# ArtoriasAbyssslayer/HashModNFFBanks-IDR

Hardware: AMD Instinct MI355X
Metric: rays/sec fwd+bwd (hash+SDF MLP) (higher is better)
Workload: dtype f32; 1 GPU; DTU-shaped synthetic uniform-sphere rays, MultiResHash L=16 T=2^19 F=2 (BASELINE.json configs[1]), full IDR training step (forward + IDRLoss + backward + clip + Adam), weights held at the geometric initialisation (lr = 0): the SURVEY.md 8(d) workload; grid_config=C2, rays_per_gpu=2048, global_rays=2048, parallelism=single GPU, world=1, ranks_seen=1, step=HIP-graph captured static-shape step

## Files before the change

### hashmodnffbanks_idr_amd/csrc/hm_trace.hip

```cpp
#include "hm_common.h"
#include "hm_trace_host.h"

#include <stdlib.h>
#include <string.h>

namespace {

constexpr int kTB = 256;

#include "hm_trace_dev.h"

__global__ __launch_bounds__(kTB) void trace_init_kernel(TraceArgs a) {
    const int64_t i = (int64_t)blockIdx.x * kTB + threadIdx.x;
    if (i >= a.n) return;
    trace_init_ray(a, i, a.w.cnt + C_ROUND0, 0);
}

__global__ __launch_bounds__(kTB) void trace_advance_kernel(TraceArgs a, int round) {
    const int64_t i = (int64_t)blockIdx.x * kTB + threadIdx.x;
    if (i >= a.n) return;
    trace_advance_ray(a, i, a.w.cnt + C_ROUND0 + round, 0);
}

__global__ __launch_bounds__(kTB) void trace_finalize_kernel(TraceArgs a) {
    const int64_t i = (int64_t)blockIdx.x * kTB + threadIdx.x;
    if (i >= a.n) return;
    const TraceWs &w = a.w;
    if (w.stage[i] != ST_DONE) atomicAdd(w.cnt + C_UNFINISHED, 1);
    const float t_s = w.t_s[i], t_e = w.t_e[i];
    a.out_mask[i] = t_s < t_e;
    a.out_t[i] = t_s;
    float px = 0.0f, py = 0.0f, pz = 0.0f;
    if (a.hit[i] || w.cnt[C_ANY_LIVE]) along(a, i, t_s, px, py, pz);
    a.out_pts[i * 3] = px; a.out_pts[i * 3 + 1] = py; a.out_pts[i * 3 + 2] = pz;
    const bool samp = w.live_s[i] != 0;
    w.is_samp[i] = samp;
    if (samp) w.list_samp[atomicAdd(w.cnt + C_NSAMP, 1)] = (int32_t)i;
}

__global__ __launch_bounds__(kTB) void ray_samples_kernel(TraceArgs a, const int32_t *list, int c_n, int c_npts,
                                                          const float *lo_arr, const float *hi_arr,
                                                          const float *fr, int c_base, int per_ray) {
    const int64_t gid = (int64_t)blockIdx.x * kTB + threadIdx.x;
    const TraceWs &w = a.w;
    const int32_t n_list = w.cnt[c_n];
    const int64_t base = c_base == -2 ? a.sel_off : (c_base >= 0 ? w.cnt[c_base] : 0);
    if (gid == 0) {
        w.cnt[c_npts] = n_list * per_ray;
        if (c_base != -2) w.cnt[C_BIG_PTS] = (int32_t)base + n_list * per_ray;
    }
    const int64_t m = gid / per_ray;
    if (m >= n_list) return;
    int s = (int)(gid - m * per_ray);
    if (per_ray < a.n_steps && s == per_ray - 1) s = a.n_steps - 1;
    const int64_t i = list[m];
    const float lo = lo_arr[i], hi = hi_arr[i];
    const float t = __fadd_rn(lo, __fmul_rn(fr[s], __fsub_rn(hi, lo)));
    float px, py, pz;
    along(a, i, t, px, py, pz);
    const int64_t o = base + gid;
    w.pts[o * 3] = px; w.pts[o * 3 + 1] = py; w.pts[o * 3 + 2] = pz;
}

__global__ __launch_bounds__(kTB) void sampler_head_kernel(TraceArgs a) {
    const int64_t m = (int64_t)blockIdx.x * kTB + threadIdx.x;
    const TraceWs &w = a.w;
    if (m >= w.cnt[C_NSAMP]) return;
    const int64_t i = w.list_samp[m];
    const float *v = w.vals + m * (a.head + 1);
    bool neg = false;
    for (int s = 0; s < a.head; ++s) neg = neg || (v[s] < 0.0f);
    const bool resolved = neg && a.obj[i] != 0;
    w.tail_slot[m] = resolved ? -1 : atomicAdd(w.cnt + C_NSAMP2, 1);
}

__global__ __launch_bounds__(kTB) void sampler_tail_points_kernel(TraceArgs a) {
    const int64_t gid = (int64_t)blockIdx.x * kTB + threadIdx.x;
    const TraceWs &w = a.w;
    const int per = a.n_steps - a.head - 1;
    if (gid == 0) {
        w.cnt[C_TAIL_PTS] = w.cnt[C_NSAMP2] * per;
        w.cnt[C_NSAMP_PTS] = w.cnt[C_HEAD_PTS] + w.cnt[C_NSAMP2] * per;
    }
    const int64_t m = gid / per;
    if (m >= w.cnt[C_NSAMP]) return;
    const int32_t q = w.tail_slot[m];
    if (q < 0) return;
    const int j = (int)(gid - m * per);
    const int64_t i = w.list_samp[m];
    const float lo = w.t_s[i], hi = w.t_e[i];
    const float t = __fadd_rn(lo, __fmul_rn(a.fracs[a.head + j], __fsub_rn(hi, lo)));
    float px, py, pz;
    along(a, i, t, px, py, pz);
    const int64_t o = a.tail_off + (int64_t)q * per + j;
    w.pts[o * 3] = px; w.pts[o * 3 + 1] = py; w.pts[o * 3 + 2] = pz;
}

__global__ __launch_bounds__(kTB) void sampler_reduce_kernel(TraceArgs a) {
    const int64_t m = (int64_t)blockIdx.x * kTB + threadIdx.x;
    const TraceWs &w = a.w;
    if (m >= w.cnt[C_NSAMP]) return;
    const int64_t i = w.list_samp[m];
    const int n = a.n_steps;
    const bool lazy = a.head > 0;
    const int32_t tq = lazy ? w.tail_slot[m] : 0;
    const float *v_head = lazy ? w.vals + m * (a.head + 1) : w.vals + m * n;
    const float *v_tail = lazy ? w.vals + a.tail_off + (int64_t)(tq < 0 ? 0 : tq) * (n - a.head - 1) - a.head : v_head;
    const int head = a.head;
    auto v = [&](int s) -> float {
        if (!lazy) return v_head[s];
        if (s < head) return v_head[s];
        return s == n - 1 ? v_head[head] : v_tail[s];
    };
    const int n_scan = (lazy && tq < 0) ? head : n;
    int first = 0, amin = 0, bad = 0;
    float best_tmp = 0.0f, best_v = 0.0f;
    auto visit = [&](int s, float x) {
        bad += !isfinite(x);
        const float sg = (x > 0.0f) ? 1.0f : ((x < 0.0f) ? -1.0f : 0.0f);
        const float tmp = sg * (float)(n - s);
        if (s == 0 || tmp < best_tmp) { best_tmp = tmp; first = s; }
        if (s == 0 || x < best_v) { best_v = x; amin = s; }
    };
    if (!lazy && (n & 3) == 0 && (reinterpret_cast<uintptr_t>(v_head) & 15u) == 0) {
        const float4 *row = reinterpret_cast<const float4 *>(v_head);
#pragma unroll 5
        for (int g4 = 0; g4 < n / 4; ++g4) {
            const float4 x4 = row[g4];
            visit(4 * g4, x4.x); visit(4 * g4 + 1, x4.y); visit(4 * g4 + 2, x4.z); visit(4 * g4 + 3, x4.w);
        }
    } else {
        for (int s = 0; s < n_scan; ++s) visit(s, v(s));
    }
    const float lo = w.t_s[i], hi = w.t_e[i];
    auto t_at = [&](int s) { return __fadd_rn(lo, __fmul_rn(a.fracs[s], __fsub_rn(hi, lo))); };
    const float v_first = v(first);
    const bool net_hit = v_first < 0.0f;
    const bool true_obj = a.obj[i] != 0;
    const int pick = (true_obj && net_hit) ? first : amin;
    float t_out = t_at(pick);
    float px, py, pz;
    along(a, i, t_out, px, py, pz);
    a.out_mask[i] = net_hit;
    const bool sec = a.training ? (net_hit && true_obj) : net_hit;
    if (sec) {
        const int lo_idx = first > 0 ? first - 1 : n - 1;
        const float z_hi = t_at(first), v_hi = v_first, z_lo = t_at(lo_idx), v_lo = v(lo_idx);
        if (lazy && tq < 0 && lo_idx == n - 1 && !isfinite(v_lo)) ++bad;
        const float z = secant_z(v_lo, v_hi, z_lo, z_hi);
        const int32_t q = atomicAdd(w.cnt + C_NSEC, 1);
        w.list_sec[q] = (int32_t)i;
        w.z_lo[q] = z_lo; w.z_hi[q] = z_hi; w.v_lo[q] = v_lo; w.v_hi[q] = v_hi; w.z[q] = z;
        if (a.n_secant == 0) {
            t_out = z;
            along(a, i, z, px, py, pz);
        }
    }
    if (bad) atomicAdd(w.cnt + C_NONFINITE, bad);
    a.out_t[i] = t_out;
    w.t_s[i] = t_out;
    a.out_pts[i * 3] = px; a.out_pts[i * 3 + 1] = py; a.out_pts[i * 3 + 2] = pz;
}

__global__ __launch_bounds__(kTB) void secant_points_kernel(TraceArgs a) {
    const int64_t q = (int64_t)blockIdx.x * kTB + threadIdx.x;
    const TraceWs &w = a.w;
    if (q >= w.cnt[C_NSEC]) return;
    float px, py, pz;
    along(a, w.list_sec[q], w.z[q], px, py, pz);
    w.pts[q * 3] = px; w.pts[q * 3 + 1] = py; w.pts[q * 3 + 2] = pz;
}

__global__ __launch_bounds__(kTB) void secant_advance_kernel(TraceArgs a, int last) {
    const int64_t q = (int64_t)blockIdx.x * kTB + threadIdx.x;
    if (q >= a.w.cnt[C_NSEC]) return;
    secant_advance_ray(a, q, last);
}

__global__ __launch_bounds__(kTB) void tail_prepare_kernel(TraceArgs a) {
    const int64_t i = (int64_t)blockIdx.x * kTB + threadIdx.x;
    if (i >= a.n) return;
    const TraceWs &w = a.w;
    const bool net = a.out_mask[i] != 0, obj = a.obj[i] != 0, samp = w.is_samp[i] != 0, hit = a.hit[i] != 0;
    const bool in_mask = !net && obj && !samp;
    const bool out_mask = !obj && !samp;
    if (!(in_mask || out_mask)) return;
    if (!hit) {
        const float *c = a.cam + (i / a.rays_per_image) * 3;
        const float *d = a.dirs + i * 3;
        const float dot = __fmaf_rn(d[2], c[2], __fmaf_rn(d[1], c[1], __fmul_rn(d[0], c[0])));
        const float t = -dot;
        float px, py, pz;
        along(a, i, t, px, py, pz);
        a.out_t[i] = t;
        w.t_s[i] = t;
        a.out_pts[i * 3] = px; a.out_pts[i * 3 + 1] = py; a.out_pts[i * 3 + 2] = pz;
        return;
    }
    if (net && out_mask) w.t_min[i] = w.t_s[i];
    w.list_sel[atomicAdd(w.cnt + C_NSEL, 1)] = (int32_t)i;
}

__global__ __launch_bounds__(kTB) void closest_reduce_kernel(TraceArgs a) {
    const int64_t m = (int64_t)blockIdx.x * kTB + threadIdx.x;
    const TraceWs &w = a.w;
    if (m >= w.cnt[C_NSEL]) return;
    const int64_t i = w.list_sel[m];
    const int n = a.n_steps;
    const float *v = w.vals + (a.sel_off >= 0 ? a.sel_off : (int64_t)w.cnt[a.head > 0 ? C_HEAD_PTS : C_NSAMP_PTS]) +
                     m * n;
    int amin = 0, bad = !isfinite(v[0]);
    float best = v[0];
    if ((n & 3) == 0 && (reinterpret_cast<uintptr_t>(v) & 15u) == 0) {
        const float4 *row = reinterpret_cast<const float4 *>(v);
        auto visit = [&](int s, float x) {
            if (s == 0) return;
            bad += !isfinite(x);
            if (x < best) { best = x; amin = s; }
        };
#pragma unroll 5
        for (int g4 = 0; g4 < n / 4; ++g4) {
            const float4 x4 = row[g4];
            visit(4 * g4, x4.x); visit(4 * g4 + 1, x4.y); visit(4 * g4 + 2, x4.z); visit(4 * g4 + 3, x4.w);
        }
    } else {
        for (int s = 1; s < n; ++s) {
            bad += !isfinite(v[s]);
            if (v[s] < best) { best = v[s]; amin = s; }
        }
    }
    if (bad) atomicAdd(w.cnt + C_NONFINITE, bad);
    const float lo = w.t_min[i], hi = w.t_max[i];
    const float t = __fadd_rn(__fmul_rn(a.steps_u[amin], __fsub_rn(hi, lo)), lo);
    float px, py, pz;
    along(a, i, t, px, py, pz);
    a.out_t[i] = t;
    a.out_pts[i * 3] = px; a.out_pts[i * 3 + 1] = py; a.out_pts[i * 3 + 2] = pz;
}

constexpr int kGuardRows = kTB / 64;
template <class V, class S, class O>
__device__ __forceinline__ void guard_mark_row(const TraceArgs &a, int lane, int n, bool signs, bool min_rule,
                                               bool true_obj, bool all, bool own_approx, bool other_approx, int c_ref,
                                               V val, S slot, O own) {
    const float tau = kGuardTau;
    const int kNone = 1 << 30;
    auto unc = [&](float x) { return !isfinite(x) || fabsf(x) <= tau; };
    int c = kNone;
    float m = INFINITY;
    for (int s = lane; s < n; s += 64) {
        const float x = val(s);
        if (signs && c == kNone && x < -tau) c = s;
        if (isfinite(x) && x < m) m = x;
    }
    for (int d = 32; d > 0; d >>= 1) {
        c = min(c, __shfl_xor(c, d));
        m = fminf(m, __shfl_xor(m, d));
    }
    const bool use_min = min_rule && (!signs || !true_obj || c == kNone);
    const float lim = m + 2.0f * tau;
    auto marked = [&](int s, float x, float xn) -> bool {
        if (!(own(s) ? own_approx : other_approx)) return false;
        if (all && own(s)) return true;
        if (!isfinite(x)) return true;
        if (use_min && x <= lim) return true;
        if (!signs) return false;
        if (fabsf(x) <= tau || s == c) return true;
        const int nx = s + 1 == n ? 0 : s + 1;
        return nx <= c && (nx == c || unc(xn));
    };
    auto mark_of = [&](int s) -> bool { return s < n && marked(s, val(s), val(s + 1 == n ? 0 : s + 1)); };
    int n_mark = 0;
    for (int s0 = 0; s0 < n; s0 += 64) n_mark += __popcll(__ballot(mark_of(s0 + lane)));
    if (n_mark == 0) return;
    int k0 = 0;
    if (lane == 0) k0 = atomicAdd(a.w.cnt + c_ref, n_mark);
    int64_t k = __shfl(k0, 0);
    for (int s0 = 0; s0 < n; s0 += 64) {
        const int s = s0 + lane;
        const bool mk = mark_of(s);
        const unsigned long long b = __ballot(mk);
        if (mk) {
            const int64_t kk = k + __popcll(b & ((1ull << lane) - 1ull));
            const int64_t o = slot(s);
            a.w.ref_slot[kk] = (int32_t)o;
            a.w.ref_pts[kk * 3] = a.w.pts[o * 3]; a.w.ref_pts[kk * 3 + 1] = a.w.pts[o * 3 + 1];
            a.w.ref_pts[kk * 3 + 2] = a.w.pts[o * 3 + 2];
        }
        k += __popcll(b);
    }
}

__global__ __launch_bounds__(kTB) void guard_select_sampler_kernel(TraceArgs a, int pass, int c_live, int c_live2,
                                                                   int64_t min_live, int c_ref) {
    const int64_t m = (int64_t)blockIdx.x * kGuardRows + (threadIdx.x >> 6);
    const int lane = threadIdx.x & 63;
    const TraceWs &w = a.w;
    if (m >= w.cnt[C_NSAMP]) return;
    const bool approx = w.cnt[c_live] >= min_live, approx2 = c_live2 >= 0 && w.cnt[c_live2] >= min_live;
    if (!approx && !approx2) return;
    const bool all = *w.guard == kGuardTripped;
    const bool true_obj = a.obj[w.list_samp[m]] != 0;
    const int n = a.n_steps, head = a.head;
    if (pass == 1) {
        const int row = head > 0 ? head + 1 : n;
        const int64_t base = m * row;
        guard_mark_row(a, lane, row, true, head == 0, true_obj, all, true, false, c_ref,
                       [&](int s) { return w.vals[base + s]; }, [&](int s) { return base + s; }, [](int) { return true; });
        return;
    }
    const int32_t tq = w.tail_slot[m];
    if (tq < 0) return;
    const int64_t b_head = m * (head + 1), b_tail = a.tail_off + (int64_t)tq * (n - head - 1) - head;
    auto slot = [&](int s) -> int64_t { return s < head ? b_head + s : (s == n - 1 ? b_head + head : b_tail + s); };
    guard_mark_row(a, lane, n, true, true, true_obj, all, approx, approx2, c_ref, [&](int s) { return w.vals[slot(s)]; },
                   slot, [&](int s) { return s >= head && s != n - 1; });
}

__global__ __launch_bounds__(kTB) void guard_select_closest_kernel(TraceArgs a, int c_live, int64_t min_live, int c_ref) {
    const int64_t m = (int64_t)blockIdx.x * kGuardRows + (threadIdx.x >> 6);
    const int lane = threadIdx.x & 63;
    const TraceWs &w = a.w;
    if (m >= w.cnt[C_NSEL] || w.cnt[c_live] < min_live) return;
    const int n = a.n_steps;
    const int64_t base = (a.sel_off >= 0 ? a.sel_off : (int64_t)w.cnt[a.head > 0 ? C_HEAD_PTS : C_NSAMP_PTS]) + m * n;
    guard_mark_row(a, lane, n, false, true, false, *w.guard == kGuardTripped, true, false, c_ref,
                   [&](int s) { return w.vals[base + s]; },
                   [&](int s) { return base + s; }, [](int) { return true; });
}

__global__ __launch_bounds__(kTB) void guard_patch_kernel(TraceArgs a, int c_ref) {
    const int64_t k = (int64_t)blockIdx.x * kTB + threadIdx.x;
    const TraceWs &w = a.w;
    const int32_t n_ref = w.cnt[c_ref];
    if (k == 0 && n_ref > 0) atomicAdd(w.cnt + C_GUARD_REFINED, n_ref);
    if (k >= n_ref) return;
    const int64_t o = w.ref_slot[k];
    const float e = w.ref_vals[k], ap = w.vals[o];
    if (isfinite(e) && isfinite(ap)) {
        const float d = fabsf(ap - e);
        if (d > 0.0f) atomicMax(w.cnt + C_GUARD_MAXDEV, __float_as_int(d));
        if (d > kGuardTrip) *w.guard = kGuardTripped;
    }
    w.vals[o] = e;
}

__global__ __launch_bounds__(kTB) void guard_noise_kernel(float *vals, int64_t off, const int32_t *n_live, int64_t min_live,
                                                          float amp, int nan_k) {
    const int64_t g = (int64_t)blockIdx.x * kTB + threadIdx.x;
    const int64_t n = *n_live;
    if (n < min_live || g >= n) return;
    const int64_t o = off + g;
    if (nan_k > 0) {
        if (o % nan_k == 0) vals[o] = ((o / nan_k) & 1) ? INFINITY : NAN;
        return;
    }
    uint32_t h = (uint32_t)o * 2654435761u;
    h ^= h >> 15; h *= 2246822519u; h ^= h >> 13;
    const float u = (float)(h >> 8) * (2.0f / 16777216.0f) - 1.0f;
    vals[o] = __fadd_rn(vals[o], __fmul_rn(amp, u));
}

__global__ void count_evals_kernel(int32_t *cnt, int rounds, int n_secant) {
    if (threadIdx.x != 0 || blockIdx.x != 0) return;
    int64_t tot = 0;
    for (int r = 0; r < rounds && r < 64; ++r) tot += cnt[C_ROUND0 + r];
    tot += cnt[C_NSAMP_PTS] + (int64_t)cnt[C_NSEC] * n_secant + cnt[C_NSEL_PTS];
    cnt[C_EVALS] = (int32_t)tot;
}

constexpr float *TraceWs::*kRayFloats[] = {&TraceWs::t_s,   &TraceWs::t_e,   &TraceWs::t_min, &TraceWs::t_max, &TraceWs::cur_s,
                                           &TraceWs::cur_e, &TraceWs::nxt_s, &TraceWs::nxt_e, &TraceWs::z_lo,  &TraceWs::z_hi,
                                           &TraceWs::v_lo,  &TraceWs::v_hi,  &TraceWs::z};
constexpr int32_t *TraceWs::*kRayInts[] = {&TraceWs::slot_s,   &TraceWs::slot_e,   &TraceWs::list_samp,
                                           &TraceWs::list_sec, &TraceWs::list_sel, &TraceWs::tail_slot};
constexpr uint8_t *TraceWs::*kRayBytes[] = {&TraceWs::live_s, &TraceWs::live_e, &TraceWs::stage,
                                            &TraceWs::it,     &TraceWs::k,      &TraceWs::is_samp};
template <class T, size_t K>
void carve_rays(HmCarve &c, TraceWs &w, T *TraceWs::*const (&members)[K], int64_t n) {
    T *p = c.take<T>((int64_t)K * n);
    for (size_t k = 0; k < K; ++k) w.*members[k] = p + (p ? (int64_t)k * n : 0);
}

constexpr int64_t kWsHeader = 256;
constexpr int kWsRegions = 3;

struct TraceLayout { TraceWs w; float *emb_ws; int64_t bytes; };
TraceLayout trace_layout(void *ws, int64_t n, int n_steps, int emb_width, bool guard) {
    TraceLayout L;
    TraceWs &w = L.w;
    HmCarve c(ws);
    w.cap = n * (n_steps > 2 ? n_steps : 2);
    w.guard = c.take<int32_t>(kWsHeader / (int64_t)sizeof(int32_t));
    carve_rays(c, w, kRayFloats, n);
    carve_rays(c, w, kRayInts, n);
    carve_rays(c, w, kRayBytes, n);
    w.pts = c.take<float>(kWsRegions * 3 * w.cap);
    w.vals = c.take<float>(kWsRegions * w.cap);
    w.cnt = c.take<int32_t>(C_COUNT);
    L.emb_ws = c.take<float>((int64_t)emb_width * w.cap);
    w.ref_pts = c.take<float>(guard ? 5 * w.cap : 0);
    w.ref_vals = w.ref_pts + (ws ? 3 * w.cap : 0);
    w.ref_slot = reinterpret_cast<int32_t *>(w.ref_vals + (ws ? w.cap : 0));
    L.bytes = c.bytes;
    return L;
}
int nffb_emb_width(int n_levels) { return 3 + 8 + 8 * n_levels; }

struct TraceSwitches {
    int overlap, chain_tiles, chain_tail;
    int tail_first;
    float noise_amp; int noise_nan;
};
TraceSwitches trace_switches() {
    const auto num = [](const char *name, int unset) {
        const char *e = getenv(name);
        return e ? atoi(e) : unset;
    };
    TraceSwitches s = {num("HM_TRACE_OVERLAP", -1), num("HM_TRACE_POOL_CHAIN_TILES", -1), num("HM_TRACE_CHAIN_TAIL", -1),
                       num("HM_TRACE_TAIL_FIRST", 0), 0.0f, 0};
    const char *e = getenv("HM_TRACE_GUARD_NOISE");
    if (e && strncmp(e, "nan:", 4) == 0) s.noise_nan = atoi(e + 4) > 0 ? atoi(e + 4) : 0;
    else if (e) { const double f_ = atof(e); if (f_ > 0.0 && f_ < 1.0) s.noise_amp = (float)(f_ * kGuardTau); }
    return s;
}

using TracePlan = hm_trace_plan_info;

TracePlan trace_plan(const hm_trace_cfg &cfg, int64_t n_rays, int tile_points, bool has_nffb, const TraceSwitches &sw) {
    TracePlan P = {};
    const bool guard = cfg.coarse_bf16 == 3;
    const int n_sec = cfg.n_secant_steps;
    const bool overlap_shape = sw.overlap != 0 && cfg.training && !has_nffb && tile_points == 0 && n_sec > 0 && n_rays <= kSdfSmall;
    const bool fill = overlap_shape && cfg.coarse_bf16 == 0;
    const bool cosched = guard && overlap_shape && sw.overlap != 1;
    const bool pooled = cosched && sw.overlap != 2;
    P.sequence = fill ? HM_TRACE_SEQ_FILL : pooled ? HM_TRACE_SEQ_GUARD_POOLED : cosched ? HM_TRACE_SEQ_GUARD_COSCHED
                 : guard ? HM_TRACE_SEQ_GUARD_SERIAL : HM_TRACE_SEQ_JOINT;
    P.sel_own = fill || (guard && overlap_shape);
    P.head = (cfg.sampler_head >= 1 && cfg.sampler_head + 1 < cfg.n_steps) ? cfg.sampler_head : 0;
    P.per_ray = P.head > 0 ? P.head + 1 : cfg.n_steps;
    P.c_first = P.head > 0 ? (int)C_HEAD_PTS : (int)C_NSAMP_PTS;
    const int tail_want = sw.chain_tail >= 0 ? sw.chain_tail : kTraceChainTail;
    P.k_tail = (pooled && tail_want > 0 && n_sec > tail_want) ? tail_want : 0;
    P.chain_tiles = pooled ? trace_chain_tiles(n_sec, sw.chain_tiles >= 0 ? sw.chain_tiles : -1) : 0;
    P.c_ref2 = (pooled && P.head > 0) ? (int)C_GUARD_N2 : -1;
    P.guard_min = tile_points == 0 ? kSdfSmall + 1 : 1;
    if (guard) { P.noise_amp = sw.noise_amp; P.noise_nan = sw.noise_nan; }
    const int64_t cap = n_rays * (cfg.n_steps > 2 ? cfg.n_steps : 2);
    P.march_rounds = 1 + cfg.sphere_tracing_iters * (1 + cfg.line_step_iters);
    P.march_tail = !has_nffb && (tile_points == 0 || tile_points == 16) && cap >= ((n_rays + 7) / 8) * 16 &&
                   cfg.line_step_iters > 0;
    P.march_launched = P.march_tail ? 1 + cfg.sphere_tracing_iters : P.march_rounds;
    if (P.march_tail && sw.tail_first >= 1 && sw.tail_first < P.march_launched) P.march_launched = sw.tail_first;
    if (n_sec == 0) P.secant = HM_TRACE_SECANT_NONE;
    else if (fill || cosched) P.secant = HM_TRACE_SECANT_IN_SEQUENCE;
    else if (!has_nffb && (tile_points == 0 || tile_points == 4 || tile_points == 8 || tile_points == 16) &&
             (tile_points != 0 || n_rays <= kSdfSmall))
        P.secant = HM_TRACE_SECANT_PERSISTENT;
    else P.secant = HM_TRACE_SECANT_PER_ITERATION;
    P.scan_rule = P.secant == HM_TRACE_SECANT_PERSISTENT && P.sel_own;
    return P;
}

struct TraceRun {
    HmTraceCtx cx; const hm_trace_cfg *cfg;
    TracePlan P; TraceArgs a;
    float *emb_ws;
    int emb_width;

    int c_samp() const { return P.sel_own ? P.c_first : (int)C_BIG_PTS; }
    int c_sel() const { return P.sel_own ? (int)C_NSEL_PTS : (int)C_BIG_PTS; }
    int64_t n_scan() const { return a.n * a.n_steps; }
    int64_t n_tail() const { return a.n * (a.n_steps - a.head - 1); }

    template <class K, class... A>
    void launch(K kernel, int64_t threads, A... args) {
        hipLaunchKernelGGL(kernel, dim3((unsigned)((threads + kTB - 1) / kTB)), dim3(kTB), 0, as_stream(cx.stream), args...);
    }
    template <class K, class... A> void per_ray(K kernel, A... args) { launch(kernel, a.n, a, args...); }
    template <class K, class... A> void per_row(K kernel, A... args) { launch(kernel, a.n * (kTB / kGuardRows), a, args...); }

    int eval(int64_t off, int64_t capacity, const int32_t *n_dev, int mode = 0) {
        const float *p = a.w.pts + off * 3;
        float *v = a.w.vals + off;
        const int64_t run_min = kSdfSmall + 1;
        const int tile = mode ? -1 : cx.tile_points;
        if (cx.nffb) {
            HM_TRY(hm_nffb_fwd(cx.desc, cx.nffb, p, capacity, cx.table, cx.B_fourier, emb_ws, emb_width, cx.frac_mode, n_dev,
                               cx.stream));
            HM_TRY(hm_sdf_fwd_emb(cx.mlp, emb_ws, emb_width, emb_width, capacity, v, 1, 1, tile, n_dev, 0, cx.stream));
            if (!mode) return HM_OK;
            return mode == 2 ? hm_sdf_fwd_emb_split(cx.mlp, emb_ws, emb_width, emb_width, capacity, v, 1, n_dev, run_min, cx.stream)
                             : hm_sdf_fwd_emb_bf16(cx.mlp, emb_ws, emb_width, emb_width, capacity, v, 1, n_dev, run_min, cx.stream);
        }
        if (mode == 3 && cx.tile_points != 0)
            return hm_sdf_fwd_split(cx.desc, cx.mlp, p, capacity, cx.table, cx.B_fourier, v, 1, cx.frac_mode, n_dev, 1, cx.stream);
        HM_TRY(hm_sdf_fwd(cx.desc, cx.mlp, p, capacity, cx.table, cx.B_fourier, v, 1, 1, cx.frac_mode, tile, n_dev, 0, cx.stream));
        if (!mode) return HM_OK;
        return mode >= 2 ? hm_sdf_fwd_split(cx.desc, cx.mlp, p, capacity, cx.table, cx.B_fourier, v, 1, cx.frac_mode, n_dev, run_min,
                                            cx.stream)
                         : hm_sdf_fwd_bf16(cx.desc, cx.mlp, p, capacity, cx.table, cx.B_fourier, v, 1, cx.frac_mode, n_dev, run_min,
                                           cx.stream);
    }
    int coarse(int64_t off, int64_t capacity, int c_live) { return eval(off, capacity, a.w.cnt + c_live, cfg->coarse_bf16); }

    void first_pass_points() {
        if (cfg->training) per_ray(tail_prepare_kernel);
        launch(ray_samples_kernel, a.n * P.per_ray, a, a.w.list_samp, (int)C_NSAMP, P.c_first, a.w.t_s, a.w.t_e, a.fracs, -1,
               P.per_ray);
        if (cfg->training)
            launch(ray_samples_kernel, n_scan(), a, a.w.list_sel, (int)C_NSEL, (int)C_NSEL_PTS, a.w.t_min, a.w.t_max, a.steps_u,
                   P.sel_own ? -2 : P.c_first, a.n_steps);
    }
    void second_pass_points() {
        per_ray(sampler_head_kernel);
        launch(sampler_tail_points_kernel, n_scan(), a);
    }

    void noise(int64_t off, int64_t capacity, int c_live) {
        if (P.noise_amp > 0.0f || P.noise_nan > 0)
            launch(guard_noise_kernel, capacity, a.w.vals, off, a.w.cnt + c_live, P.guard_min, P.noise_amp, P.noise_nan);
    }
    void select_sampler(int pass, int c_live, int c_live2, int c_ref) {
        per_row(guard_select_sampler_kernel, pass, c_live, c_live2, P.guard_min, c_ref);
    }
    void select_closest(int c_live, int c_ref) { per_row(guard_select_closest_kernel, c_live, P.guard_min, c_ref); }
    int refine(int c_ref, bool quarter = false) {
        return hm_sdf_fwd(cx.desc, cx.mlp, a.w.ref_pts, a.w.cap, cx.table, cx.B_fourier, a.w.ref_vals, 1, 1, cx.frac_mode,
                          cx.tile_points == 0 ? (quarter ? HM_SDF_TILE64_QUARTER : 64) : cx.tile_points, a.w.cnt + c_ref, 0,
                          cx.stream);
    }
    int refine_beside_scan(int which) {
        return hm_trace_refine_scan(&cx, &a, C_GUARD_N1, P.c_ref2, which, a.sel_off, n_scan(), P.chain_tiles);
    }
    void patch(int c_ref) { launch(guard_patch_kernel, a.w.cap, a, c_ref); }
    int second_pass() {
        if (a.head == 0) return HM_OK;
        second_pass_points();
        HM_TRY(coarse(a.tail_off, n_tail(), C_TAIL_PTS));
        if (cfg->coarse_bf16 != 3) return HM_OK;
        noise(a.tail_off, n_tail(), C_TAIL_PTS);
        select_sampler(2, C_TAIL_PTS, c_samp(), C_GUARD_N2);
        HM_TRY(P.c_ref2 >= 0 ? refine_beside_scan(1) : refine(C_GUARD_N2));
        patch(C_GUARD_N2);
        return HM_OK;
    }
    int sampler_beside_scan() {
        HM_TRY(coarse(0, n_scan(), c_samp()));
        noise(0, n_scan(), c_samp());
        select_sampler(1, c_samp(), -1, C_GUARD_N1);
        HM_TRY(refine_beside_scan(0));
        patch(C_GUARD_N1);
        HM_TRY(second_pass());
        per_ray(sampler_reduce_kernel);
        per_ray(secant_points_kernel);
        return HM_OK;
    }
    template <class F>
    int closest_rows_own_list(F refine_launch) {
        noise(a.sel_off, n_scan(), C_NSEL_PTS);
        select_closest(C_NSEL_PTS, C_GUARD_NC);
        HM_TRY(refine_launch());
        patch(C_GUARD_NC);
        per_ray(closest_reduce_kernel);
        return HM_OK;
    }
    int secant_beside_list(int it_first, int n_iters, int quarter) {
        return hm_trace_scan_secant(&cx, &a, it_first, n_iters, a.n_secant, quarter, a.w.ref_pts, a.w.ref_vals, a.w.cap,
                                    C_GUARD_NC, 0, -1, 0, -1, 0);
    }
    int reduce_and_secant() {
        per_ray(sampler_reduce_kernel);
        if (P.secant == HM_TRACE_SECANT_NONE) return HM_OK;
        per_ray(secant_points_kernel);
        if (P.secant == HM_TRACE_SECANT_PERSISTENT) return hm_trace_secant_persistent(&cx, &a, a.n_secant, P.scan_rule);
        for (int s = 0; s < a.n_secant; ++s) {
            HM_TRY(eval(0, a.n, a.w.cnt + C_NSEC));
            per_ray(secant_advance_kernel, s == a.n_secant - 1 ? 1 : 0);
        }
        return HM_OK;
    }

    int march() {
        per_ray(trace_init_kernel);
        for (int r = 0; r < P.march_launched; ++r) {
            HM_TRY(eval(0, 2 * a.n, a.w.cnt + C_ROUND0 + r));
            per_ray(trace_advance_kernel, r + 1 < 64 ? r + 1 : 63);
        }
        if (P.march_tail) HM_TRY(hm_trace_march_tail(&cx, &a, P.march_launched, P.march_rounds));
        per_ray(trace_finalize_kernel);
        return HM_OK;
    }

    int seq_joint() {
        HM_TRY(coarse(0, n_scan(), C_BIG_PTS));
        if (cfg->training) per_ray(closest_reduce_kernel);
        HM_TRY(second_pass());
        return reduce_and_secant();
    }
    int seq_fill() {
        int grid_p1 = 0, grid_p2 = 0;
        const float *x_fill = a.w.pts + a.sel_off * 3;
        float *out_fill = a.w.vals + a.sel_off;
        HM_TRY(hm_sdf_fwd_fill(&cx, a.w.pts, n_scan(), a.w.vals, a.w.cnt + P.c_first, x_fill, out_fill, a.w.cnt + C_NSEL_PTS,
                               nullptr, 0, &grid_p1));
        if (a.head > 0) {
            second_pass_points();
            HM_TRY(hm_sdf_fwd_fill(&cx, a.w.pts + a.tail_off * 3, n_tail(), a.w.vals + a.tail_off, a.w.cnt + C_TAIL_PTS, x_fill,
                                   out_fill, a.w.cnt + C_NSEL_PTS, a.w.cnt + P.c_first, grid_p1, &grid_p2));
        }
        per_ray(sampler_reduce_kernel);
        per_ray(secant_points_kernel);
        HM_TRY(hm_trace_scan_secant(&cx, &a, 0, a.n_secant, a.n_secant, 0, x_fill, out_fill, n_scan(), C_NSEL_PTS, 1, P.c_first,
                                    grid_p1, C_TAIL_PTS, grid_p2));
        per_ray(closest_reduce_kernel);
        return HM_OK;
    }
    int seq_guard_serial() {
        HM_TRY(coarse(0, n_scan(), c_samp()));
        if (P.sel_own) HM_TRY(coarse(a.sel_off, n_scan(), c_sel()));
        noise(0, n_scan(), c_samp());
        if (P.sel_own) noise(a.sel_off, n_scan(), c_sel());
        select_sampler(1, c_samp(), -1, C_GUARD_N1);
        if (cfg->training) select_closest(c_sel(), C_GUARD_N1);
        HM_TRY(refine(C_GUARD_N1));
        patch(C_GUARD_N1);
        if (cfg->training) per_ray(closest_reduce_kernel);
        HM_TRY(second_pass());
        return reduce_and_secant();
    }
    int seq_guard_cosched() {
        HM_TRY(sampler_beside_scan());
        return closest_rows_own_list([&] { return secant_beside_list(0, a.n_secant, 0); });
    }
    int seq_guard_pooled() {
        const int n_front = a.n_secant - P.k_tail;
        HM_TRY(sampler_beside_scan());
        HM_TRY(hm_trace_split_scan_secant(&cx, &a, 0, n_front, a.n_secant, C_GUARD_N1, P.c_ref2, a.sel_off, n_scan(),
                                          P.chain_tiles));
        return closest_rows_own_list(
            [&] { return P.k_tail > 0 ? secant_beside_list(n_front, P.k_tail, 1) : refine(C_GUARD_NC, true); });
    }

    int run(int32_t *stats_out) {
        hm_zero_u32_async(a.w.cnt, C_COUNT, as_stream(cx.stream));
        HM_TRY(march());
        first_pass_points();
        switch (P.sequence) {
        case HM_TRACE_SEQ_FILL: HM_TRY(seq_fill()); break;
        case HM_TRACE_SEQ_GUARD_SERIAL: HM_TRY(seq_guard_serial()); break;
        case HM_TRACE_SEQ_GUARD_COSCHED: HM_TRY(seq_guard_cosched()); break;
        case HM_TRACE_SEQ_GUARD_POOLED: HM_TRY(seq_guard_pooled()); break;
        default: HM_TRY(seq_joint()); break;
        }
        hipLaunchKernelGGL(count_evals_kernel, dim3(1), dim3(64), 0, as_stream(cx.stream), a.w.cnt, P.march_rounds + 1, a.n_secant);
        if (stats_out)
            hipLaunchKernelGGL(hm_copy_u32_kernel, dim3(1), dim3(64), 0, as_stream(cx.stream), reinterpret_cast<uint32_t *>(stats_out),
                               reinterpret_cast<const uint32_t *>(a.w.cnt + C_NSAMP), 16);
        HM_CHECK_LAUNCH("hm_trace_forward");
        return HM_OK;
    }
};

}

extern "C" {

int64_t hm_trace_workspace_bytes(int64_t n_rays, const hm_trace_cfg *cfg) {
    if (n_rays < 0 || !cfg || cfg->n_steps < 1) return hm_fail(HM_ERR_INVALID, "hm_trace_workspace_bytes: bad argument");
    return trace_layout(nullptr, n_rays, cfg->n_steps, 0, cfg->coarse_bf16 == 3).bytes;
}

int hm_trace_guard_clear(void *workspace, int64_t workspace_bytes, void *stream) {
    HM_CHECK_ARG(workspace && workspace_bytes >= kWsHeader, "hm_trace_guard_clear: no workspace");
    hm_zero_u32_async(reinterpret_cast<int32_t *>(workspace), kWsHeader / sizeof(int32_t), as_stream(stream));
    HM_CHECK_LAUNCH("hm_trace_guard_clear");
    return HM_OK;
}

int hm_trace_guard_tolerances(float *tau, float *tau_trip) {
    HM_CHECK_ARG(tau && tau_trip, "hm_trace_guard_tolerances: NULL pointer");
    *tau = kGuardTau;
    *tau_trip = kGuardTrip;
    return HM_OK;
}

int64_t hm_trace_workspace_bytes_nffb(int64_t n_rays, const hm_trace_cfg *cfg, int n_levels) {
    if (n_rays < 0 || !cfg || cfg->n_steps < 1 || n_levels < 1 || n_levels > HM_MAX_LEVELS)
        return hm_fail(HM_ERR_INVALID, "hm_trace_workspace_bytes_nffb: bad argument");
    return trace_layout(nullptr, n_rays, cfg->n_steps, nffb_emb_width(n_levels), false).bytes;
}

int hm_diag_trace_plan(int64_t n_rays, const hm_trace_cfg *cfg, int tile_points, int has_nffb, hm_trace_plan_info *info) {
    HM_CHECK_ARG(n_rays >= 0 && cfg && info && cfg->n_steps >= 2, "hm_diag_trace_plan: bad argument");
    *info = trace_plan(*cfg, n_rays, tile_points, has_nffb != 0, trace_switches());
    return HM_OK;
}

static int trace_forward_impl(const HmTraceCtx &cx, const hm_trace_cfg *cfg, const float *cam_loc, const float *ray_dirs,
                              const uint8_t *object_mask, const float *t_sphere, const uint8_t *hit_mask, int64_t n_rays,
                              int64_t rays_per_image, const float *sampler_fracs, const float *steps_u, float *out_points,
                              uint8_t *out_net_mask, float *out_dists, void *workspace, int64_t workspace_bytes,
                              int32_t *stats_out) {
    HM_CHECK_ARG(cx.desc && cx.mlp && cfg, "hm_trace_forward: NULL descriptor");
    HM_CHECK_ARG(n_rays >= 0 && rays_per_image >= 1, "hm_trace_forward: bad ray counts");
    HM_CHECK_ARG(cfg->n_steps >= 2 && cfg->n_steps <= 4096, "hm_trace_forward: n_steps out of range");
    HM_CHECK_ARG(cfg->sphere_tracing_iters >= 0 && cfg->sphere_tracing_iters <= 15 && cfg->line_step_iters >= 0 &&
                     cfg->line_step_iters <= 3 &&
                     1 + cfg->sphere_tracing_iters * (1 + cfg->line_step_iters) <= 64,
                 "hm_trace_forward: too many march rounds (sphere_tracing_iters <= 15, line_step_iters <= 3)");
    HM_CHECK_ARG(cfg->n_secant_steps >= 0 && cfg->n_secant_steps <= 64, "hm_trace_forward: n_secant_steps out of range");
    if (n_rays == 0) return HM_OK;
    HM_CHECK_ARG(n_rays * (int64_t)cfg->n_steps < (1ll << 31), "hm_trace_forward: too many rays for one call");
    HM_CHECK_ARG(cx.table && cx.B_fourier && cam_loc && ray_dirs && object_mask && t_sphere && hit_mask && sampler_fracs &&
                     out_points && out_net_mask && out_dists && workspace,
                 "hm_trace_forward: NULL pointer");
    HM_CHECK_ARG(!cfg->training || steps_u, "hm_trace_forward: training mode needs steps_u");
    HM_CHECK_ARG(cfg->coarse_bf16 >= 0 && cfg->coarse_bf16 <= 3, "hm_trace_forward: coarse_bf16 must be 0, 1, 2 or 3");
    const bool guard = cfg->coarse_bf16 == 3;
    HM_CHECK_ARG(!guard || !cx.nffb, "hm_trace_forward: the guarded coarse scans do not cover filter-bank embedders");
    HM_CHECK_ARG(!guard || 3 * n_rays * (int64_t)cfg->n_steps < (1ll << 31), "hm_trace_forward: too many rays for one call");
    TraceRun R;
    R.cx = cx; R.cfg = cfg;
    R.P = trace_plan(*cfg, n_rays, cx.tile_points, cx.nffb != nullptr, trace_switches());
    R.emb_width = cx.nffb ? nffb_emb_width(cx.nffb->n_levels) : 0;
    const TraceLayout L = trace_layout(workspace, n_rays, cfg->n_steps, R.emb_width, guard);
    HM_CHECK_ARG(workspace_bytes >= L.bytes, "hm_trace_forward: workspace too small");
    R.emb_ws = L.emb_ws;
    TraceArgs &a = R.a;
    a.w = L.w;
    a.cam = cam_loc; a.dirs = ray_dirs; a.obj = object_mask; a.t_sphere = t_sphere; a.hit = hit_mask;
    a.fracs = sampler_fracs; a.steps_u = steps_u;
    a.out_pts = out_points; a.out_mask = out_net_mask; a.out_t = out_dists;
    a.n = n_rays; a.rays_per_image = rays_per_image;
    a.thr = cfg->sdf_threshold;
    for (int k = 0; k < 4; ++k) a.back[k] = (float)((1.0 - cfg->line_search_step) / (double)(1 << k));
    a.ls_iters = cfg->line_step_iters; a.max_it = cfg->sphere_tracing_iters; a.n_steps = cfg->n_steps;
    a.n_secant = cfg->n_secant_steps; a.training = cfg->training;
    a.head = R.P.head;
    a.tail_off = a.w.cap;
    a.sel_off = R.P.sel_own ? 2 * a.w.cap : -1;
    return R.run(stats_out);
}

int hm_trace_forward(const hm_grid_desc *desc, const hm_mlp_desc *mlp, const float *table, const float *B_fourier,
                     int frac_mode, int tile_points, const hm_trace_cfg *cfg, const float *cam_loc,
                     const float *ray_dirs, const uint8_t *object_mask, const float *t_sphere,
                     const uint8_t *hit_mask, int64_t n_rays, int64_t rays_per_image, const float *sampler_fracs,
                     const float *steps_u, float *out_points, uint8_t *out_net_mask, float *out_dists,
                     void *workspace, int64_t workspace_bytes, int32_t *stats_out, void *stream) {
    return trace_forward_impl({desc, nullptr, mlp, table, B_fourier, frac_mode, tile_points, stream}, cfg, cam_loc, ray_dirs,
                              object_mask, t_sphere, hit_mask, n_rays, rays_per_image, sampler_fracs, steps_u, out_points,
                              out_net_mask, out_dists, workspace, workspace_bytes, stats_out);
}

int hm_trace_forward_nffb(const hm_grid_desc *desc, const hm_nffb_desc *nffb, const hm_mlp_desc *mlp, const float *table,
                          const float *B_fourier, int frac_mode, int tile_points, const hm_trace_cfg *cfg,
                          const float *cam_loc, const float *ray_dirs, const uint8_t *object_mask, const float *t_sphere,
                          const uint8_t *hit_mask, int64_t n_rays, int64_t rays_per_image, const float *sampler_fracs,
                          const float *steps_u, float *out_points, uint8_t *out_net_mask, float *out_dists,
                          void *workspace, int64_t workspace_bytes, int32_t *stats_out, void *stream) {
    HM_CHECK_ARG(nffb != nullptr, "hm_trace_forward_nffb: NULL embedder descriptor");
    return trace_forward_impl({desc, nffb, mlp, table, B_fourier, frac_mode, tile_points, stream}, cfg, cam_loc, ray_dirs,
                              object_mask, t_sphere, hit_mask, n_rays, rays_per_image, sampler_fracs, steps_u, out_points,
                              out_net_mask, out_dists, workspace, workspace_bytes, stats_out);
}

}
```

Measured before the change: 334,300 rays/s.

## Fuse small ray-tracing kernels to cut launches in the sphere-trace pipeline

Folds tail_prepare into trace_finalize, computes secant points inside sampler_reduce instead of a separate kernel, merges the two ray_samples launches into one grid, and folds the stats copy into a warp-reduced count_evals kernel. The aim is fewer tiny kernel launches and dependent passes per training step inside the captured graph. Risks: ordering changes (tail_prepare now runs before later stages that previously preceded it, e.g. list_sel fill timing), and count_evals now caps rounds at 64 lanes via a shuffle reduction.

Measured after the change: 334,800 rays/s (median of 6 runs). No clear change (+0.1%).

```diff
diff --git a/hashmodnffbanks_idr_amd/csrc/hm_trace.hip b/hashmodnffbanks_idr_amd/csrc/hm_trace.hip
--- a/hashmodnffbanks_idr_amd/csrc/hm_trace.hip
+++ b/hashmodnffbanks_idr_amd/csrc/hm_trace.hip
@@ -22,13 +22,36 @@
     trace_advance_ray(a, i, a.w.cnt + C_ROUND0 + round, 0);
 }
 
+__device__ __forceinline__ void tail_prepare_ray(const TraceArgs &a, int64_t i, bool net, bool samp, float t_s) {
+    const TraceWs &w = a.w;
+    const bool obj = a.obj[i] != 0, hit = a.hit[i] != 0;
+    const bool in_mask = !net && obj && !samp;
+    const bool out_mask = !obj && !samp;
+    if (!(in_mask || out_mask)) return;
+    if (!hit) {
+        const float *c = a.cam + (i / a.rays_per_image) * 3;
+        const float *d = a.dirs + i * 3;
+        const float dot = __fmaf_rn(d[2], c[2], __fmaf_rn(d[1], c[1], __fmul_rn(d[0], c[0])));
+        const float t = -dot;
+        float px, py, pz;
+        along(a, i, t, px, py, pz);
+        a.out_t[i] = t;
+        w.t_s[i] = t;
+        a.out_pts[i * 3] = px; a.out_pts[i * 3 + 1] = py; a.out_pts[i * 3 + 2] = pz;
+        return;
+    }
+    if (net && out_mask) w.t_min[i] = t_s;
+    w.list_sel[atomicAdd(w.cnt + C_NSEL, 1)] = (int32_t)i;
+}
+
 __global__ __launch_bounds__(kTB) void trace_finalize_kernel(TraceArgs a) {
     const int64_t i = (int64_t)blockIdx.x * kTB + threadIdx.x;
     if (i >= a.n) return;
     const TraceWs &w = a.w;
     if (w.stage[i] != ST_DONE) atomicAdd(w.cnt + C_UNFINISHED, 1);
     const float t_s = w.t_s[i], t_e = w.t_e[i];
-    a.out_mask[i] = t_s < t_e;
+    const bool net = t_s < t_e;
+    a.out_mask[i] = net;
     a.out_t[i] = t_s;
     float px = 0.0f, py = 0.0f, pz = 0.0f;
     if (a.hit[i] || w.cnt[C_ANY_LIVE]) along(a, i, t_s, px, py, pz);
@@ -36,12 +59,12 @@
     const bool samp = w.live_s[i] != 0;
     w.is_samp[i] = samp;
     if (samp) w.list_samp[atomicAdd(w.cnt + C_NSAMP, 1)] = (int32_t)i;
-}
-
-__global__ __launch_bounds__(kTB) void ray_samples_kernel(TraceArgs a, const int32_t *list, int c_n, int c_npts,
-                                                          const float *lo_arr, const float *hi_arr,
-                                                          const float *fr, int c_base, int per_ray) {
-    const int64_t gid = (int64_t)blockIdx.x * kTB + threadIdx.x;
+    if (a.training) tail_prepare_ray(a, i, net, samp, t_s);
+}
+
+__device__ __forceinline__ void ray_samples(const TraceArgs &a, int64_t gid, const int32_t *list, int c_n, int c_npts,
+                                            const float *lo_arr, const float *hi_arr, const float *fr, int c_base,
+                                            int per_ray) {
     const TraceWs &w = a.w;
     const int32_t n_list = w.cnt[c_n];
     const int64_t base = c_base == -2 ? a.sel_off : (c_base >= 0 ? w.cnt[c_base] : 0);
@@ -60,6 +83,19 @@
     along(a, i, t, px, py, pz);
     const int64_t o = base + gid;
     w.pts[o * 3] = px; w.pts[o * 3 + 1] = py; w.pts[o * 3 + 2] = pz;
+}
+__global__ __launch_bounds__(kTB) void ray_samples_kernel(TraceArgs a, const int32_t *list, int c_n, int c_npts,
+                                                          const float *lo_arr, const float *hi_arr,
+                                                          const float *fr, int c_base, int per_ray) {
+    ray_samples(a, (int64_t)blockIdx.x * kTB + threadIdx.x, list, c_n, c_npts, lo_arr, hi_arr, fr, c_base, per_ray);
+}
+__global__ __launch_bounds__(kTB) void ray_samples_both_kernel(TraceArgs a, int blocks_samp, int c_first, int per_ray) {
+    const int64_t b = blockIdx.x;
+    if (b < blocks_samp)
+        ray_samples(a, b * kTB + threadIdx.x, a.w.list_samp, C_NSAMP, c_first, a.w.t_s, a.w.t_e, a.fracs, -1, per_ray);
+    else
+        ray_samples(a, (b - blocks_samp) * kTB + threadIdx.x, a.w.list_sel, C_NSEL, C_NSEL_PTS, a.w.t_min, a.w.t_max,
+                    a.steps_u, -2, a.n_steps);
 }
 
 __global__ __launch_bounds__(kTB) void sampler_head_kernel(TraceArgs a) {
@@ -151,9 +187,13 @@
         const int32_t q = atomicAdd(w.cnt + C_NSEC, 1);
         w.list_sec[q] = (int32_t)i;
         w.z_lo[q] = z_lo; w.z_hi[q] = z_hi; w.v_lo[q] = v_lo; w.v_hi[q] = v_hi; w.z[q] = z;
+        float mx, my, mz;
+        along(a, i, z, mx, my, mz);
         if (a.n_secant == 0) {
             t_out = z;
-            along(a, i, z, px, py, pz);
+            px = mx; py = my; pz = mz;
+        } else {
+            w.pts[(int64_t)q * 3] = mx; w.pts[(int64_t)q * 3 + 1] = my; w.pts[(int64_t)q * 3 + 2] = mz;
         }
     }
     if (bad) atomicAdd(w.cnt + C_NONFINITE, bad);
@@ -162,43 +202,10 @@
     a.out_pts[i * 3] = px; a.out_pts[i * 3 + 1] = py; a.out_pts[i * 3 + 2] = pz;
 }
 
-__global__ __launch_bounds__(kTB) void secant_points_kernel(TraceArgs a) {
-    const int64_t q = (int64_t)blockIdx.x * kTB + threadIdx.x;
-    const TraceWs &w = a.w;
-    if (q >= w.cnt[C_NSEC]) return;
-    float px, py, pz;
-    along(a, w.list_sec[q], w.z[q], px, py, pz);
-    w.pts[q * 3] = px; w.pts[q * 3 + 1] = py; w.pts[q * 3 + 2] = pz;
-}
-
 __global__ __launch_bounds__(kTB) void secant_advance_kernel(TraceArgs a, int last) {
     const int64_t q = (int64_t)blockIdx.x * kTB + threadIdx.x;
     if (q >= a.w.cnt[C_NSEC]) return;
     secant_advance_ray(a, q, last);
-}
-
-__global__ __launch_bounds__(kTB) void tail_prepare_kernel(TraceArgs a) {
-    const int64_t i = (int64_t)blockIdx.x * kTB + threadIdx.x;
-    if (i >= a.n) return;
-    const TraceWs &w = a.w;
-    const bool net = a.out_mask[i] != 0, obj = a.obj[i] != 0, samp = w.is_samp[i] != 0, hit = a.hit[i] != 0;
-    const bool in_mask = !net && obj && !samp;
-    const bool out_mask = !obj && !samp;
-    if (!(in_mask || out_mask)) return;
-    if (!hit) {
-        const float *c = a.cam + (i / a.rays_per_image) * 3;
-        const float *d = a.dirs + i * 3;
-        const float dot = __fmaf_rn(d[2], c[2], __fmaf_rn(d[1], c[1], __fmul_rn(d[0], c[0])));
-        const float t = -dot;
-        float px, py, pz;
-        along(a, i, t, px, py, pz);
-        a.out_t[i] = t;
-        w.t_s[i] = t;
-        a.out_pts[i * 3] = px; a.out_pts[i * 3 + 1] = py; a.out_pts[i * 3 + 2] = pz;
-        return;
-    }
-    if (net && out_mask) w.t_min[i] = w.t_s[i];
-    w.list_sel[atomicAdd(w.cnt + C_NSEL, 1)] = (int32_t)i;
 }
 
 __global__ __launch_bounds__(kTB) void closest_reduce_kernel(TraceArgs a) {
@@ -361,12 +368,13 @@
     vals[o] = __fadd_rn(vals[o], __fmul_rn(amp, u));
 }
 
-__global__ void count_evals_kernel(int32_t *cnt, int rounds, int n_secant) {
-    if (threadIdx.x != 0 || blockIdx.x != 0) return;
-    int64_t tot = 0;
-    for (int r = 0; r < rounds && r < 64; ++r) tot += cnt[C_ROUND0 + r];
+__global__ __launch_bounds__(64) void count_evals_kernel(int32_t *cnt, int rounds, int n_secant, int32_t *stats_out) {
+    const int lane = threadIdx.x;
+    int64_t tot = lane < rounds ? cnt[C_ROUND0 + lane] : 0;
+    for (int d = 32; d > 0; d >>= 1) tot += __shfl_xor(tot, d);
     tot += cnt[C_NSAMP_PTS] + (int64_t)cnt[C_NSEC] * n_secant + cnt[C_NSEL_PTS];
-    cnt[C_EVALS] = (int32_t)tot;
+    if (lane == 0) cnt[C_EVALS] = (int32_t)tot;
+    if (stats_out && lane < 16) stats_out[lane] = C_NSAMP + lane == C_EVALS ? (int32_t)tot : cnt[C_NSAMP + lane];
 }
 
 constexpr float *TraceWs::*kRayFloats[] = {&TraceWs::t_s,   &TraceWs::t_e,   &TraceWs::t_min, &TraceWs::t_max, &TraceWs::cur_s,
@@ -506,7 +514,11 @@
     int coarse(int64_t off, int64_t capacity, int c_live) { return eval(off, capacity, a.w.cnt + c_live, cfg->coarse_bf16); }
 
     void first_pass_points() {
-        if (cfg->training) per_ray(tail_prepare_kernel);
+        if (cfg->training && P.sel_own) {
+            const int64_t blocks_samp = (a.n * P.per_ray + kTB - 1) / kTB;
+            launch(ray_samples_both_kernel, blocks_samp * kTB + n_scan(), a, (int)blocks_samp, P.c_first, P.per_ray);
+            return;
+        }
         launch(ray_samples_kernel, a.n * P.per_ray, a, a.w.list_samp, (int)C_NSAMP, P.c_first, a.w.t_s, a.w.t_e, a.fracs, -1,
                P.per_ray);
         if (cfg->training)
@@ -554,7 +566,6 @@
         patch(C_GUARD_N1);
         HM_TRY(second_pass());
         per_ray(sampler_reduce_kernel);
-        per_ray(secant_points_kernel);
         return HM_OK;
     }
     template <class F>
@@ -573,7 +584,6 @@
     int reduce_and_secant() {
         per_ray(sampler_reduce_kernel);
         if (P.secant == HM_TRACE_SECANT_NONE) return HM_OK;
-        per_ray(secant_points_kernel);
         if (P.secant == HM_TRACE_SECANT_PERSISTENT) return hm_trace_secant_persistent(&cx, &a, a.n_secant, P.scan_rule);
         for (int s = 0; s < a.n_secant; ++s) {
             HM_TRY(eval(0, a.n, a.w.cnt + C_NSEC));
@@ -611,7 +621,6 @@
                                    out_fill, a.w.cnt + C_NSEL_PTS, a.w.cnt + P.c_first, grid_p1, &grid_p2));
         }
         per_ray(sampler_reduce_kernel);
-        per_ray(secant_points_kernel);
         HM_TRY(hm_trace_scan_secant(&cx, &a, 0, a.n_secant, a.n_secant, 0, x_fill, out_fill, n_scan(), C_NSEL_PTS, 1, P.c_first,
                                     grid_p1, C_TAIL_PTS, grid_p2));
         per_ray(closest_reduce_kernel);
@@ -654,10 +663,8 @@
         case HM_TRACE_SEQ_GUARD_POOLED: HM_TRY(seq_guard_pooled()); break;
         default: HM_TRY(seq_joint()); break;
         }
-        hipLaunchKernelGGL(count_evals_kernel, dim3(1), dim3(64), 0, as_stream(cx.stream), a.w.cnt, P.march_rounds + 1, a.n_secant);
-        if (stats_out)
-            hipLaunchKernelGGL(hm_copy_u32_kernel, dim3(1), dim3(64), 0, as_stream(cx.stream), reinterpret_cast<uint32_t *>(stats_out),
-                               reinterpret_cast<const uint32_t *>(a.w.cnt + C_NSAMP), 16);
+        hipLaunchKernelGGL(count_evals_kernel, dim3(1), dim3(64), 0, as_stream(cx.stream), a.w.cnt, P.march_rounds + 1, a.n_secant,
+                           stats_out);
         HM_CHECK_LAUNCH("hm_trace_forward");
         return HM_OK;
     }
```
